# prtk1729/Paligemma-MultiModal-System

Measured on AMD Instinct MI355X. Metric: image→text tokens/sec + prefill ms, PaliGemma-3B-224 at 1/2/4/8 MI355X, higher is better.
Workload: dtype bf16; 1 GPU; PaliGemma-3B-pt-224 image->text, batch 1, prefill L=264, 128 greedy tokens (BASELINE.json configs[1]); global_batch=1, seq_len=392, parallelism=dp1, decode=hipgraph, prefill=eager

## Files before the change

### paligemma-multimodal-system_amd/csrc/common.h

```cpp
#pragma once
#include <hip/hip_runtime.h>
#include <stdint.h>

typedef uint16_t bf16_t;
typedef __attribute__((ext_vector_type(8))) __bf16 bf16x8;
typedef __attribute__((ext_vector_type(4))) float f32x4;
typedef __attribute__((ext_vector_type(2))) float f32x2;
typedef __attribute__((ext_vector_type(4))) uint32_t u32x4;
typedef __attribute__((ext_vector_type(2))) uint32_t u32x2;

#define LDS_AS __attribute__((address_space(3)))

__device__ __forceinline__ float bf2f(bf16_t v) { return __uint_as_float(((uint32_t)v) << 16); }

__device__ __forceinline__ bf16_t f2bf(float f) {
  __bf16 b = (__bf16)f;
  return __builtin_bit_cast(bf16_t, b);
}
typedef __bf16 pg_bf16x2_t __attribute__((ext_vector_type(2)));
typedef float pg_f32x2_t __attribute__((ext_vector_type(2)));
__device__ __forceinline__ uint32_t pack_bf2(float lo, float hi) {
  return __builtin_bit_cast(uint32_t, __builtin_convertvector(pg_f32x2_t{lo, hi}, pg_bf16x2_t));
}

__device__ __forceinline__ float bf_lo(uint32_t v) { return __uint_as_float(v << 16); }
__device__ __forceinline__ float bf_hi(uint32_t v) { return __uint_as_float(v & 0xffff0000u); }
__device__ __forceinline__ uint32_t pack_fp8x4(float a, float b, float c, float d) {
  int w = __builtin_amdgcn_cvt_pk_fp8_f32(fminf(fmaxf(a, -448.f), 448.f), fminf(fmaxf(b, -448.f), 448.f), 0, false);
  w = __builtin_amdgcn_cvt_pk_fp8_f32(fminf(fmaxf(c, -448.f), 448.f), fminf(fmaxf(d, -448.f), 448.f), w, true);
  return (uint32_t)w;
}

__device__ __forceinline__ float max_xor16(float v) {
  const auto r = __builtin_amdgcn_permlane16_swap(__float_as_uint(v), __float_as_uint(v), false, false);
  return fmaxf(__uint_as_float(r[0]), __uint_as_float(r[1]));
}
__device__ __forceinline__ float max_xor32(float v) {
  const auto r = __builtin_amdgcn_permlane32_swap(__float_as_uint(v), __float_as_uint(v), false, false);
  return fmaxf(__uint_as_float(r[0]), __uint_as_float(r[1]));
}
__device__ __forceinline__ float sum_xor16(float v) {
  const auto r = __builtin_amdgcn_permlane16_swap(__float_as_uint(v), __float_as_uint(v), false, false);
  return __uint_as_float(r[0]) + __uint_as_float(r[1]);
}
// ... 112 lines not shown
```

### paligemma-multimodal-system_amd/csrc/gemm.hip

```cpp
#include "gemm_common.h"

static int gemm_impl(const void* A, int lda, const void* W, int ldw, const float* bias, void* C, int ldc,
                     int M, int N, int K, int epi_flags, int ksplit, const float* aux, int aux_rows, void* aux_out,
                     int aux_ld, int aux_n, const PgFusedArgs* fa, hipStream_t stream) {
  const bool frag = (epi_flags & PG_W_FRAG) != 0;
  const bool fp8 = (epi_flags & PG_FP8) != 0;
  const bool m1 = (epi_flags & PG_TILE_M1) != 0;
  const bool n64 = (epi_flags & PG_TILE_N64) != 0;
  const int epi = epi_flags & 0xFF;
  const bool slot_rows = (epi_flags & PG_SLOT_ROWS) != 0;
  const bool frag13 = (epi_flags & PG_W_FRAG13) != 0;
  const bool frag12 = (epi_flags & PG_W_FRAG12) != 0;
  PG_REQUIRE((epi_flags & ~(0xFF | PG_W_FRAG | PG_FP8 | PG_TILE_M1 | PG_TILE_N64 | PG_SLOT_ROWS | PG_W_FRAG13 |
                            PG_W_FRAG12)) == 0 &&
             epi <= PG_EPI_F32_RES && (frag13 || !frag12));
  if (frag13) {
    const int pm = fa ? fa->pro_mode : 0;
    PG_REQUIRE(!frag && !fp8 && !m1 && !n64 && W != nullptr && ((uintptr_t)W & 15) == 0 && M >= 1 && M <= 4 &&
               N > 0 && N % 16 == 0 && K > 0 && K % 128 == 0 && ldw == K && ksplit >= 1 && ksplit <= 64 &&
               (K / 64) % (8 * ksplit) == 0);
    PG_REQUIRE((epi == PG_EPI_QKV_ROPE && pm == 1) || (epi == PG_EPI_BF16_GELU_MUL && pm == 1) ||
               (epi == PG_EPI_FX_ADD && (pm == 0 || pm == 2)) || (epi == PG_EPI_F32_FIN && pm == 0) ||
               (epi == PG_EPI_F32 && pm == 4));
  }
  if (m1) PG_REQUIRE(!fp8 && !n64 && M >= 256 && M <= 288 && (fa == nullptr || fa->pro_mode == 0));
  if (n64) PG_REQUIRE(M > 16);
  PG_REQUIRE(M > 0 && N > 0 && K > 0 && ksplit >= 1 && W != nullptr && C != nullptr);
  PG_REQUIRE(K % 32 == 0 && ldw >= K && (N % 4) == 0);
  if (frag && !fp8) PG_REQUIRE(N % 16 == 0 && K % 64 == 0 && ldw == K &&
                       (epi == PG_EPI_BF16 || epi == PG_EPI_BF16_GELU_MUL || epi == PG_EPI_F32 ||
                        epi == PG_EPI_QKV_ROPE || epi == PG_EPI_F32_FIN || epi == PG_EPI_F32_ADD ||
                        epi == PG_EPI_FX_ADD || epi == PG_EPI_F32_RES));
  PgFusedArgs f{};
// ... 98 lines not shown
```

### paligemma-multimodal-system_amd/csrc/gemm_gemv.hip

```cpp
#include "gemm_common.h"

#define XPAD 8

#ifndef PG_GEMV_PREW
#define PG_GEMV_PREW 1
#endif
#ifndef PG_GEMV_NT
#define PG_GEMV_NT 0
#endif
#ifndef PG_GEMV_CONTIG
#define PG_GEMV_CONTIG 0
#endif
#ifndef PG_GEMV_QKV_NT1
#define PG_GEMV_QKV_NT1 1
#endif
#ifndef PG_GEMV_D2
#define PG_GEMV_D2 4
#endif
#ifndef PG_GEMV_LM_NT
#define PG_GEMV_LM_NT 2
#endif
#ifndef PG_GEMV_LM_D
#define PG_GEMV_LM_D 6
#endif
// ... 300 lines not shown
  u32x4 cq;
  unsigned c5;
};
template <int MODE>
__device__ __forceinline__ void decode12(const W12& b, unsigned bias, u32x4 (&op)[2][2]) {
  unsigned q[4] = {b.cq[0], b.cq[1], b.cq[2], b.cq[3]};
  unsigned c5 = 0;
#pragma unroll
  for (int d = 0; d < 4; ++d) asm volatile("" : "+v"(q[d]));
  if constexpr (MODE > 0) {
    c5 = b.c5;
    asm volatile("" : "+v"(c5));
  }
  const unsigned badd = bias * 0x00800080u;
#pragma unroll
  for (int P = 0; P < 16; ++P) {
    const unsigned w = q[P >> 2];
    unsigned e = ((P & 3) == 0 ? w << 7 : (P & 3) == 1 ? w << 3 : (P & 3) == 2 ? w >> 1 : w >> 5) & 0x07800780u;
    if constexpr (MODE > 0)
      e |= (P < 11 ? c5 << (11 - P) : c5 >> (P - 11)) & 0x08000800u;
    if constexpr (MODE == 2) {
      const unsigned nz = ((e + 0x0f800f80u) >> 5) & 0x00800080u;
      e += __umul24(nz, bias);
    } else {
      e += badd;
    }
    const int h = P >> 3, s = (P >> 2) & 1, p = P & 3;
    const unsigned x = b.sm[h][p];
    const unsigned d = __builtin_amdgcn_perm(x, x, s == 0 ? 0x02020000u : 0x03030101u);
    op[h][s][p] = (d & 0x807f807fu) | e;
  }
}

template <int EPI, int NT, int U, int DEPTH, int PRO, int FRAG, int CPW = 0>
__device__ __forceinline__ void gemv_body(const bf16_t* __restrict__ A, int lda, const bf16_t* __restrict__ W,
                                          int ldw, int K, const EpiArgs& e, const GemvIdx gi) {
  constexpr int CH = U * 32;
  extern __shared__ __attribute__((aligned(16))) char dyn_smem[];
  const int lane = threadIdx.x & 63;
  const int wave = threadIdx.x >> 6;
  const int g = lane >> 4;
  const int r = lane & 15;
  const int tile0 = gi.bx * NT;
  const int M = e.M;
  const bool xvalid = r < M;

  const int z = gi.by;
  const int nch_all = K / CH;
  const int per_z = (nch_all + gi.ny - 1) / gi.ny;
  const int c0 = z * per_z;
  const int nch = min(nch_all - c0, per_z);
  const int mine = CPW > 0 ? CPW : (nch > wave ? (nch - wave + 3) / 4 : 0);
  constexpr int DB = DEPTH / 2;
  const int nb = CPW > 0 ? CPW / 2 : nch >> 3;

  const bf16_t* wrow[NT];
  const bf16_t* wfrag[NT];
#pragma unroll
  for (int t = 0; t < NT; ++t) {
    int n = (tile0 + t) * 16 + r;
    n = n < e.N ? n : e.N - 1;
    wrow[t] = W + (size_t)n * ldw;
    wfrag[t] = W + (size_t)min(tile0 + t, (e.N >> 4) - 1) * 16 * ldw;
  }
  f32x4 acc[NT];
#pragma unroll
  for (int t = 0; t < NT; ++t) acc[t] = f32x4{0.f, 0.f, 0.f, 0.f};

  bf16_t* xs = (bf16_t*)dyn_smem;
  const int Kr = per_z * CH;
  const bf16_t* xrow = (PRO == 0 || PRO == 4) ? A + (size_t)(xvalid ? r : M - 1) * lda : nullptr;
  constexpr bool SS16 = PRO == 4 && (NT >= 2 || EPI == PG_EPI_QKV_ROPE);
  constexpr int SSL = SS16 ? 16 : 4;
  float ssv[SSL];
#pragma unroll
  for (int k = 0; k < SSL; ++k) ssv[k] = 0.f;
  if constexpr (PRO == 4) {
    if (wave == 0) {
      if (SS16 && M > 2) {
        const int rr = min(r, M - 1);
#pragma unroll
        for (int k = 0; k < SSL; ++k) ssv[k] = e.f.ss_in[(size_t)rr * e.f.ss_ld + min(g + 4 * k, e.f.ss_n - 1)];
      } else {
        const int lpr = M == 1 ? 64 : 32;
        const int rr = min(lane / lpr, M - 1);
#pragma unroll
        for (int k = 0; k < 4; ++k) ssv[k] = e.f.ss_in[(size_t)rr * e.f.ss_ld + min(lane % lpr + k * lpr, e.f.ss_n - 1)];
      }
    }
  }
  const bf16_t* xlds = xs + (xvalid ? r : M - 1) * (Kr + XPAD);
  int rope_p = 0, rope_slot_raw = 0;
  if constexpr (EPI == PG_EPI_QKV_ROPE) {
    rope_p = e.f.pos[r < M ? r : M - 1];
    const int* slot_p = e.f.slot_dev ? e.f.slot_dev : &pg_zero_word;
    if (e.slot_rows) slot_p += (r < M ? r : M - 1) / e.f.rows_per_batch;
    rope_slot_raw = __hip_atomic_load(slot_p, __ATOMIC_RELAXED, __HIP_MEMORY_SCOPE_AGENT);
  }

  constexpr int S_STRIDE = PG_GEMV_CONTIG ? 32 : 8;
  const int LANE_OFF = PG_GEMV_CONTIG ? g * 8 : g * 8 * U;
  u32x4 wb[FRAG >= 2 ? 1 : DEPTH][NT][U];
  u32x4 xb[DEPTH][U];
  W13 wc[FRAG == 2 ? DB : 1][NT];
  constexpr int NTW = CPW > 0 ? CPW / 2 : DB;
  W12 wd[FRAG == 3 ? DB : 1][NT];
  unsigned tw[FRAG == 3 ? NT : 1][FRAG == 3 ? NTW : 1];
  unsigned twv[FRAG == 3 && CPW > 0 ? NT : 1][FRAG == 3 && CPW > 0 ? NTW : 1];
  const char* const w12 = (const char*)W;
  const size_t nblk12 = (size_t)(e.N >> 4) * (K >> 7);
  const unsigned* const tab12 = (const unsigned*)(w12 + nblk12 * PG_F12_BLOCK);
  const char* const heap12 = (const char*)tab12 + ((nblk12 * 4 + 255) & ~(size_t)255);
  auto blk12 = [&](int t, int i) {
    return (size_t)min(tile0 + t, (e.N >> 4) - 1) * (K >> 7) + ((c0 >> 3) + i) * 4 + wave;
  };
  if constexpr (FRAG == 3 && CPW > 0) {
#pragma unroll
    for (int i = 0; i < NTW; ++i)
#pragma unroll
      for (int t = 0; t < NT; ++t) twv[t][i] = tab12[blk12(t, i)];
    __builtin_amdgcn_sched_barrier(0);
  }
  auto loadm12 = [&](int i, W12 (&wv)[NT]) {
// ... 169 lines not shown
    float* scratch = (float*)(dyn_smem + (((size_t)M * (Kr + XPAD) * 2 + 15) & ~(size_t)15));
    if (PRO == 1 && PG_GEMV_PRO_EARLY && early)
      pro1_row_finish(e.f, K, p1, xs, scratch);
    else
      gemv_prologue<PRO>(e, M, K, c0 * CH, nch * CH, xs, scratch, A, lda, gi);
  }
#pragma unroll
  for (int d = 0; d < DEPTH; ++d) {
    if constexpr (FRAG == 2) {
      if (d < DB && (CPW > 0 ? d < CPW / 2 : d < nb)) {
        if (!prew) loadw13(d, wc[d]);
        loadx(2 * d, xb[2 * d]);
        loadx(2 * d + 1, xb[2 * d + 1]);
      }
      __builtin_amdgcn_sched_barrier(0);
    } else if constexpr (FRAG == 3) {
      if (d < DB && (CPW > 0 ? d < CPW / 2 : d < nb)) {
        if (!prew) {
          if constexpr (CPW > 0) loadm12(d, wd[d]);
          else loadw12(d, d, wd[d]);
        }
        loadx(2 * d, xb[2 * d]);
        loadx(2 * d + 1, xb[2 * d + 1]);
      }
      __builtin_amdgcn_sched_barrier(0);
    } else if (CPW > 0 ? d < CPW : d < mine) {
      if (!prew) loadw(d, wb[d]);
      loadx(d, xb[d]);
    }
  }
  if constexpr (FRAG == 3 && CPW > 0) {
    if (!prew) fifth12();
  }
  f32x4 fin_r[NT], fin_w[NT];
  i64x2 fin_fa[NT], fin_fb[NT];
  if constexpr (EPI == PG_EPI_F32_FIN) {
#pragma unroll
    for (int t = 0; t < NT; ++t) {
      const int n0 = min((tile0 + t) * 16, e.N - 16) + 4 * g;
      const size_t ro = (size_t)(r < M ? r : M - 1) * e.N + n0;
      fin_r[t] = *(const f32x4*)(e.f.fin_resid + ro);
      const long long* p = e.f.fx ? e.f.fx + ro : (const long long*)e.f.fin_resid;
      fin_fa[t] = *(const i64x2*)p;
      fin_fb[t] = *(const i64x2*)(p + 2);
      fin_w[t] = *(const f32x4*)((e.f.norm_w ? e.f.norm_w : e.f.fin_resid) + n0);
    }
  }
  f32x4 rope_cs[NT], rope_sn[NT];
  if constexpr (EPI == PG_EPI_QKV_ROPE) {
#pragma unroll
    for (int t = 0; t < NT; ++t) {
      bool roped;
      const int ii = rope_freq_index(e.f, min((tile0 + t) * 16, e.N - 16) + 4 * g, &roped);
      const long off = (long)rope_p * (e.f.head_dim >> 1) + ii;
      rope_cs[t] = *(const f32x4*)(e.f.cos_t + off);
      rope_sn[t] = *(const f32x4*)(e.f.sin_t + off);
    }
  }
  if constexpr (FRAG == 2 && CPW > 0) {
    __builtin_amdgcn_sched_barrier(0);
#pragma unroll
    for (int i = 0; i < CPW / 2; ++i) {
      const int d = i % DB;
      mfma13(wc[d], xb[2 * d], xb[2 * d + 1]);
      if (i + DB < CPW / 2) {
        loadw13(i + DB, wc[d]);
// ... 249 lines not shown
          if (e.bias && z == 0) v += load4_guard(e.bias, n0, e.N);
          if (e.f.resid_in && z == 0) v += load4_guard(e.f.resid_in + (size_t)m * e.N, n0, e.N);
          unsigned long long* dst = (unsigned long long*)e.C + (size_t)m * e.ldc + n0;
#pragma unroll
          for (int j = 0; j < 4; ++j) atomicAdd(dst + j, (unsigned long long)fx_from_f32_checked(v[j], e.f.status));
        }
      }
    }
    return;
  }
  if constexpr (EPI == PG_EPI_BF16_GELU_MUL) {
#pragma unroll
    for (int t = 0; t < NT; t += 2) epi_gelu_mul4(e, m, (tile0 + t) * 16, q, acc[t], acc[t + 1]);
  } else if constexpr (EPI == PG_EPI_QKV_ROPE) {
#pragma unroll
    for (int t = 0; t < NT; ++t) {
      f32x4 v = acc[t];
      const int n0 = (tile0 + t) * 16 + q;
      if (e.bias && n0 < e.N) v += load4_guard(e.bias, n0, e.N);
      f32x4 pr;
#pragma unroll
      for (int j = 0; j < 4; ++j) pr[j] = xchg_xor32(v[j]);
      epi_qkv_rope4_core(e, m, n0, v, pr, rope_cs[t], rope_sn[t], e.f.slot_base + rope_slot_raw);
    }
  } else {
#pragma unroll
    for (int t = 0; t < NT; ++t) epi_store4<EPI>(e, m, (tile0 + t) * 16 + q, acc[t], z);
  }
}

template <int EPI, int NT, int U, int DEPTH, int PRO, int FRAG, int CPW = 0>
__global__ __launch_bounds__(256)
__attribute__((amdgpu_waves_per_eu(FRAG >= 2 && CPW > 0 && EPI == PG_EPI_BF16_GELU_MUL ? 4 : 1, 8)))
void gemv_kernel(const bf16_t* __restrict__ A, int lda,
                                                   const bf16_t* __restrict__ W, int ldw, int K, EpiArgs e) {
  gemv_body<EPI, NT, U, DEPTH, PRO, FRAG, CPW>(A, lda, W, ldw, K, e,
                                               GemvIdx{(int)blockIdx.x, (int)blockIdx.y, (int)gridDim.x, (int)gridDim.y});
}

template <int EPI, int NT, int DEPTH, int PRO, bool FRAG>
static void launch_gemv_cpw(dim3 grid, size_t lds, hipStream_t st, const bf16_t* A, int lda, const bf16_t* W, int ldw,
                            int K, int ksplit, const EpiArgs& e) {
  const int nch = K / 64;
  const int cpw = (nch % ksplit == 0 && (nch / ksplit) % 4 == 0) ? nch / ksplit / 4 : 0;
  switch (PG_GEMV_CPW ? cpw : 0) {
    case 4: hipLaunchKernelGGL((gemv_kernel<EPI, NT, 2, DEPTH, PRO, FRAG, 4>), grid, dim3(256), lds, st, A, lda, W, ldw, K, e); break;
    case 8: hipLaunchKernelGGL((gemv_kernel<EPI, NT, 2, DEPTH, PRO, FRAG, 8>), grid, dim3(256), lds, st, A, lda, W, ldw, K, e); break;
    case 16: hipLaunchKernelGGL((gemv_kernel<EPI, NT, 2, DEPTH, PRO, FRAG, 16>), grid, dim3(256), lds, st, A, lda, W, ldw, K, e); break;
    default: hipLaunchKernelGGL((gemv_kernel<EPI, NT, 2, DEPTH, PRO, FRAG, 0>), grid, dim3(256), lds, st, A, lda, W, ldw, K, e); break;
  }
}

template <int EPI, int PRO, bool FRAG>
static void launch_gemv_pro(const bf16_t* A, int lda, const bf16_t* W, int ldw, int K, int ksplit, const EpiArgs& e,
                            hipStream_t st) {
  const int ntiles = (e.N + 15) / 16;
  const int CH = 64;
  const int per_z = (K / CH + ksplit - 1) / ksplit;
  size_t lds = 0;
  if ((PRO != 0 && PRO != 4) || PG_GEMV_XLDS) {
    lds = (size_t)e.M * (per_z * CH + XPAD) * 2;
    lds = (lds + 15) & ~(size_t)15;
    if (PRO == 1) lds += 64 * sizeof(float);
    if (PRO == 3) lds += 80 * sizeof(float);
  }
  if constexpr (PG_GEMV_QKV_NT1 && EPI == PG_EPI_QKV_ROPE) {
    if (e.M > 4) {
      launch_gemv_cpw<EPI, 1, PG_GEMV_D2, PRO, FRAG>(dim3(ntiles, ksplit), lds, st, A, lda, W, ldw, K, ksplit, e);
      return;
    }
  }
  if constexpr (PG_GEMV_LM_NT == 2 && EPI == PG_EPI_F32) {
    if (e.M <= 4 && ntiles >= 8192 && ksplit == 1) {
      launch_gemv_cpw<EPI, 2, PG_GEMV_LM_D, PRO, FRAG>(dim3((ntiles + 1) / 2, 1), lds, st, A, lda, W, ldw, K, 1, e);
      return;
    }
  }
  if constexpr (PG_GEMV_FIN_NT == 4 && EPI == PG_EPI_F32_FIN) {
    if (e.M > 4 && ntiles % 4 == 0) {
      launch_gemv_cpw<EPI, 4, PG_GEMV_D2, PRO, FRAG>(dim3(ntiles / 4, ksplit), lds, st, A, lda, W, ldw, K, ksplit, e);
      return;
    }
// ... 7 lines not shown

template <int EPI, bool FRAG>
static void launch_gemv(const bf16_t* A, int lda, const bf16_t* W, int ldw, int K, int ksplit, const EpiArgs& e,
                        hipStream_t st) {
  if constexpr (EPI == PG_EPI_F32_ADD || EPI == PG_EPI_FX_ADD) {
    if (e.f.pro_mode == 2)
      launch_gemv_pro<EPI, 2, FRAG>(A, lda, W, ldw, K, ksplit, e, st);
    else
      launch_gemv_pro<EPI, 0, FRAG>(A, lda, W, ldw, K, ksplit, e, st);
    return;
  }
  switch (e.f.pro_mode) {
    case 1: launch_gemv_pro<EPI, 1, FRAG>(A, lda, W, ldw, K, ksplit, e, st); break;
    case 2: launch_gemv_pro<EPI, 2, FRAG>(A, lda, W, ldw, K, ksplit, e, st); break;
    case 3: launch_gemv_pro<EPI, 3, FRAG>(A, lda, W, ldw, K, ksplit, e, st); break;
    case 4: launch_gemv_pro<EPI, 4, FRAG>(A, lda, W, ldw, K, ksplit, e, st); break;
    default: launch_gemv_pro<EPI, 0, FRAG>(A, lda, W, ldw, K, ksplit, e, st); break;
  }
}

template <int EPI, int NT, int DEPTH, int PRO, int F>
static void launch_gemv13(const bf16_t* A, int lda, const void* W, int K, int ksplit, const EpiArgs& e, hipStream_t st) {
  static_assert(DEPTH % 2 == 0, "whole blocks in flight");
  const int ntiles = e.N / 16;
  const int per_z = K / 64 / ksplit;
  size_t lds = 0;
  if (PRO != 0 && PRO != 4) {
    lds = (size_t)e.M * (per_z * 64 + XPAD) * 2;
    lds = (lds + 15) & ~(size_t)15;
    if (PRO == 1) lds += 64 * sizeof(float);
  }
  const dim3 grid((ntiles + NT - 1) / NT, ksplit);
  const bf16_t* w = (const bf16_t*)W;
  switch (PG_GEMV_CPW ? per_z / 4 : 0) {
    case 4: hipLaunchKernelGGL((gemv_kernel<EPI, NT, 2, DEPTH, PRO, F, 4>), grid, dim3(256), lds, st, A, lda, w, K, K, e); break;
    case 8: hipLaunchKernelGGL((gemv_kernel<EPI, NT, 2, DEPTH, PRO, F, 8>), grid, dim3(256), lds, st, A, lda, w, K, K, e); break;
    default: hipLaunchKernelGGL((gemv_kernel<EPI, NT, 2, DEPTH, PRO, F, 0>), grid, dim3(256), lds, st, A, lda, w, K, K, e); break;
  }
}

template <int F>
static int dispatch_gemv13(int epi, const bf16_t* A, int lda, const void* W, int K, int ksplit, const EpiArgs& e,
                           hipStream_t st) {
  const int pm = e.f.pro_mode;
  if (e.M > 4 || (K / 64) % (8 * ksplit)) return (int)hipErrorInvalidValue;
  if (epi == PG_EPI_QKV_ROPE && pm == 1) launch_gemv13<PG_EPI_QKV_ROPE, 1, PG_GEMV_D1, 1, F>(A, lda, W, K, ksplit, e, st);
  else if (epi == PG_EPI_FX_ADD && pm == 2) launch_gemv13<PG_EPI_FX_ADD, 1, PG_GEMV_D1, 2, F>(A, lda, W, K, ksplit, e, st);
  else if (epi == PG_EPI_FX_ADD && pm == 0) launch_gemv13<PG_EPI_FX_ADD, 1, PG_GEMV_D1, 0, F>(A, lda, W, K, ksplit, e, st);
  else if (epi == PG_EPI_F32_FIN && pm == 0) launch_gemv13<PG_EPI_F32_FIN, 1, PG_GEMV_D1, 0, F>(A, lda, W, K, ksplit, e, st);
  else if (epi == PG_EPI_BF16_GELU_MUL && pm == 1)
    launch_gemv13<PG_EPI_BF16_GELU_MUL, 2, PG_GEMV_D2, 1, F>(A, lda, W, K, ksplit, e, st);
  else if (epi == PG_EPI_F32 && pm == 4) launch_gemv13<PG_EPI_F32, 2, PG_GEMV_LM_D, 4, F>(A, lda, W, K, ksplit, e, st);
  else return (int)hipErrorInvalidValue;
  return 0;
}

int pg_dispatch_gemv13(int epi, int bits, const bf16_t* A, int lda, const void* W, int K, int ksplit, const EpiArgs& e,
                       hipStream_t st) {
  return bits == 12 ? dispatch_gemv13<3>(epi, A, lda, W, K, ksplit, e, st)
                    : dispatch_gemv13<2>(epi, A, lda, W, K, ksplit, e, st);
}

int pg_dispatch_gemv(int epi, bool frag, const bf16_t* A, int lda, const bf16_t* W, int ldw, int K, int ksplit,
                     const EpiArgs& e, hipStream_t st) {
#define PG_CASE(E)                                                                             \
  case E:                                                                                      \
    if (frag) launch_gemv<E, true>(A, lda, W, ldw, K, ksplit, e, st);                          \
    else launch_gemv<E, false>(A, lda, W, ldw, K, ksplit, e, st);                              \
    return 0;
#define PG_CASE_ROWMAJOR(E)                                                                    \
// ... 18 lines not shown
```

### paligemma-multimodal-system_amd/csrc/misc.hip

```cpp
#include <cstdlib>

#include "common.h"

__global__ void im2col_kernel(const float* __restrict__ px, int B, int C, int H, int W, int p, int nh, int nw,
                              bf16_t* __restrict__ out, int ldk) {
  const long total = (long)B * nh * nw * ldk;
  for (long i = blockIdx.x * (long)blockDim.x + threadIdx.x; i < total; i += (long)gridDim.x * blockDim.x) {
    const int col = (int)(i % ldk);
    const long row = i / ldk;
    const int pw = (int)(row % nw);
    const int ph = (int)((row / nw) % nh);
    const int b = (int)(row / ((long)nw * nh));
    float v = 0.f;
    if (col < C * p * p) {
      const int c = col / (p * p), kh = (col / p) % p, kw = col % p;
      v = px[(((long)b * C + c) * H + ph * p + kh) * W + pw * p + kw];
    }
    out[i] = f2bf(v);
  }
}

extern "C" int pg_patch_im2col(const float* px, int B, int C, int H, int W, int p, void* out, int ldk,
                               hipStream_t stream) {
  PG_REQUIRE(px && out && B > 0 && C > 0 && p > 0 && ldk >= C * p * p && H >= p && W >= p);
// ... 132 lines not shown
    vtc[((long)b * KV + cidx) * Smax + slot] = v[cidx];
}

extern "C" int pg_rope_kv_write(void* qkv, int ldq, const int* pos, int T, int L, int Hq, int Hkv, int D,
                                const float* cosT, const float* sinT, void* kc, void* vtc, int Smax, int slot_base,
                                const int* slot_dev, hipStream_t stream) {
  PG_REQUIRE(qkv && pos && cosT && sinT && kc && vtc && T > 0 && L > 0 && T % L == 0 && D % 2 == 0);
  hipLaunchKernelGGL(rope_kv_kernel, dim3(T), dim3(256), 0, stream, (bf16_t*)qkv, ldq, pos, L, Hq, Hkv, D, cosT, sinT,
                     (bf16_t*)kc, (bf16_t*)vtc, Smax, slot_base, slot_dev);
  PG_LAUNCH_CHECK();
  return 0;
}

#define AM_CHUNKS 64
__device__ __forceinline__ void am_better(float& bv, int& bi, float v, int i) {
  if (v > bv || (v == bv && i < bi)) { bv = v; bi = i; }
}
#define AM_NONE 0x7FFFFFFF
__device__ __forceinline__ int am_id(int bi) { return bi == AM_NONE ? 0 : bi; }
__device__ __forceinline__ void am_block(float& bv, int& bi, float* sv, int* si) {
  const int lane = threadIdx.x & 63, w = threadIdx.x >> 6;
#pragma unroll
  for (int o = 32; o > 0; o >>= 1) {
    float ov = __shfl_xor(bv, o, 64);
    int oi = __shfl_xor(bi, o, 64);
    am_better(bv, bi, ov, oi);
  }
  if (lane == 0) { sv[w] = bv; si[w] = bi; }
  __syncthreads();
  bv = sv[0]; bi = si[0];
  for (int i = 1; i < (int)(blockDim.x >> 6); ++i) am_better(bv, bi, sv[i], si[i]);
}

__global__ __launch_bounds__(256) void argmax_partial_kernel(const float* __restrict__ x, long ld, int V,
                                                             float* __restrict__ pv, int* __restrict__ pi) {
  __shared__ float sv[4];
  __shared__ int si[4];
  const int b = blockIdx.y, ch = blockIdx.x;
  const int per = ((V + AM_CHUNKS - 1) / AM_CHUNKS + 3) & ~3;
  const int s = ch * per, e = min(V, s + per);
  const float* row = x + (long)b * ld;
  float bv = -INFINITY;
  int bi = AM_NONE;
  for (int i = s + threadIdx.x * 4; i < e; i += 1024) {
    if (i + 3 < e) {
      const f32x4 v = *(const f32x4*)(row + i);
#pragma unroll
      for (int j = 0; j < 4; ++j) am_better(bv, bi, v[j], i + j);
    } else {
      for (int j = 0; j < 4 && i + j < e; ++j) am_better(bv, bi, row[i + j], i + j);
    }
  }
  am_block(bv, bi, sv, si);
  if (threadIdx.x == 0) { pv[b * AM_CHUNKS + ch] = bv; pi[b * AM_CHUNKS + ch] = bi; }
}

__global__ __launch_bounds__(1024) void argmax_final_kernel(const float* __restrict__ pv, const int* __restrict__ pi,
                                                            int B, int64_t* __restrict__ out_ids, int64_t* __restrict__ hist,
                                                            int hist_rows, int* __restrict__ step, int* __restrict__ pos,
                                                            int* __restrict__ kv_len) {
  const int lane = threadIdx.x & 63, wave = threadIdx.x >> 6, nw = blockDim.x >> 6;
  const int st = step ? *step : 0;
  __syncthreads();
  for (int b = wave; b < B; b += nw) {
    float bv = pv[b * AM_CHUNKS + lane];
    int bi = pi[b * AM_CHUNKS + lane];
#pragma unroll
    for (int o = 32; o > 0; o >>= 1) {
      float ov = __shfl_xor(bv, o, 64);
      int oi = __shfl_xor(bi, o, 64);
      am_better(bv, bi, ov, oi);
    }
    if (lane == 0) {
      bi = am_id(bi);
      out_ids[b] = bi;
      if (hist && st < hist_rows) hist[(long)st * B + b] = bi;
      if (pos) pos[b] += 1;
    }
  }
  if (threadIdx.x == 0) {
    if (kv_len) *kv_len += 1;
    if (step) *step = st + 1;
  }
}

#define AM_EMB_MAX_B 1024
struct AmEmbArgs {
  const bf16_t* embed;
  int V, n_feat, H;
  const float* feat;
  int64_t image_id, pad_id;
  float img_scale, normalizer;
  float* res;
};
__global__ __launch_bounds__(1024) void argmax_final_embed_kernel(const float* __restrict__ pv, const int* __restrict__ pi,
                                                                  int B, int64_t* __restrict__ out_ids,
                                                                  int64_t* __restrict__ hist, int hist_rows,
                                                                  int* __restrict__ step, int* __restrict__ pos,
                                                                  int* __restrict__ kv_len, AmEmbArgs ea) {
  __shared__ int win[AM_EMB_MAX_B];
  const int lane = threadIdx.x & 63, wave = threadIdx.x >> 6, nw = blockDim.x >> 6;
  const int st = step ? *step : 0;
  for (int b = wave; b < B; b += nw) {
    float bv = pv[b * AM_CHUNKS + lane];
    int bi = pi[b * AM_CHUNKS + lane];
#pragma unroll
    for (int o = 32; o > 0; o >>= 1) {
      float ov = __shfl_xor(bv, o, 64);
      int oi = __shfl_xor(bi, o, 64);
      am_better(bv, bi, ov, oi);
    }
    if (lane == 0) {
      bi = am_id(bi);
      win[b] = bi;
      out_ids[b] = bi;
      if (hist && st < hist_rows) hist[(long)st * B + b] = bi;
      if (pos) pos[b] += 1;
    }
  }
  __syncthreads();
  if (threadIdx.x == 0) {
    if (kv_len) *kv_len += 1;
    if (step) *step = st + 1;
  }
  for (int b = wave; b < B; b += nw) {
    const int64_t id = win[b];
    int rk = 0;
    if (id == ea.image_id)
      for (int i = 0; i < b; ++i) rk += win[i] == ea.image_id;
    embed_row(ea.res + (long)b * ea.H, id, rk, lane, 64, ea.embed, ea.V, ea.feat, ea.n_feat, ea.H, ea.image_id,
              ea.pad_id, ea.img_scale, ea.normalizer);
  }
// ... 11 lines not shown
    for (int o = 32; o > 0; o >>= 1) {
      float ov = __shfl_xor(bv, o, 64);
      int oi = __shfl_xor(bi, o, 64);
      am_better(bv, bi, ov, oi);
    }
    if (lane == 0) { pairs[2 * b] = bi == AM_NONE ? NAN : bv; pairs[2 * b + 1] = (float)(am_id(bi) + vocab_offset); }
  }
}

__global__ void argmax_merge_kernel(const float* __restrict__ pairs, int world, int B, int64_t* __restrict__ out_ids,
                                    int64_t* __restrict__ hist, int hist_rows, int* __restrict__ step, int* __restrict__ pos,
                                    int* __restrict__ kv_len) {
  if (threadIdx.x != 0) return;
  const int st = step ? *step : 0;
  for (int b = 0; b < B; ++b) {
    float bv = -INFINITY;
    int bi = AM_NONE;
    for (int r = 0; r < world; ++r) am_better(bv, bi, pairs[(r * B + b) * 2], (int)pairs[(r * B + b) * 2 + 1]);
    bi = am_id(bi);
    out_ids[b] = bi;
    if (hist && st < hist_rows) hist[(long)st * B + b] = bi;
    if (pos) pos[b] += 1;
  }
  if (kv_len) *kv_len += 1;
  if (step) *step = st + 1;
}

extern "C" int pg_argmax_pairs(const float* logits, long ld, int B, int V, int vocab_offset, void* workspace,
                               float* pairs, hipStream_t stream) {
  PG_REQUIRE(logits && workspace && pairs && B > 0 && V > 0 && ld % 4 == 0 && vocab_offset >= 0 &&
             vocab_offset + V < (1 << 24));
  float* pv = (float*)workspace;
  int* pi = (int*)(pv + B * AM_CHUNKS);
  hipLaunchKernelGGL(argmax_partial_kernel, dim3(AM_CHUNKS, B), dim3(256), 0, stream, logits, ld, V, pv, pi);
  hipLaunchKernelGGL(argmax_pairs_kernel, dim3(1), dim3(64 * am_waves(B)), 0, stream, pv, pi, B, vocab_offset, pairs);
  PG_LAUNCH_CHECK();
  return 0;
}

extern "C" int pg_argmax_merge(const float* pairs, int world, int B, int64_t* out_ids, int64_t* hist, int hist_rows,
                               int* step, int* pos, int* kv_len, hipStream_t stream) {
  PG_REQUIRE(pairs && out_ids && world > 0 && B > 0 && (hist == nullptr || hist_rows > 0));
  hipLaunchKernelGGL(argmax_merge_kernel, dim3(1), dim3(64), 0, stream, pairs, world, B, out_ids, hist, hist_rows,
                     step, pos, kv_len);
  PG_LAUNCH_CHECK();
  return 0;
}

extern "C" int pg_argmax(const float* logits, long ld, int B, int V, void* workspace, int64_t* out_ids,
                         int64_t* hist, int hist_rows, int* step, int* pos, int* kv_len, hipStream_t stream) {
  PG_REQUIRE(logits && workspace && out_ids && B > 0 && V > 0 && ld % 4 == 0 && (hist == nullptr || hist_rows > 0));
  float* pv = (float*)workspace;
  int* pi = (int*)(pv + B * AM_CHUNKS);
  hipLaunchKernelGGL(argmax_partial_kernel, dim3(AM_CHUNKS, B), dim3(256), 0, stream, logits, ld, V, pv, pi);
  hipLaunchKernelGGL(argmax_final_kernel, dim3(1), dim3(64 * am_waves(B)), 0, stream, pv, pi, B, out_ids, hist, hist_rows, step, pos,
                     kv_len);
  PG_LAUNCH_CHECK();
  return 0;
}

extern "C" int pg_argmax_embed(const float* logits, long ld, int B, int V, void* workspace, int64_t* out_ids,
                               int64_t* hist, int hist_rows, int* step, int* pos, int* kv_len, const void* embed,
                               int V_embed, const float* feat, int n_feat, int H, long image_id, long pad_id,
                               float img_scale, float normalizer, float* res, hipStream_t stream) {
  PG_REQUIRE(logits && workspace && out_ids && B > 0 && B <= AM_EMB_MAX_B && V > 0 && ld % 4 == 0 &&
             (hist == nullptr || hist_rows > 0));
  PG_REQUIRE(embed != nullptr && res != nullptr && V_embed > 0 && H > 0 && H % 4 == 0 && (n_feat == 0 || feat));
  float* pv = (float*)workspace;
  int* pi = (int*)(pv + B * AM_CHUNKS);
  const AmEmbArgs ea{(const bf16_t*)embed, V_embed, n_feat, H, feat, (int64_t)image_id, (int64_t)pad_id,
                     img_scale, normalizer, res};
  hipLaunchKernelGGL(argmax_partial_kernel, dim3(AM_CHUNKS, B), dim3(256), 0, stream, logits, ld, V, pv, pi);
  hipLaunchKernelGGL(argmax_final_embed_kernel, dim3(1), dim3(64 * am_waves(B)), 0, stream, pv, pi, B, out_ids, hist,
                     hist_rows, step, pos, kv_len, ea);
  PG_LAUNCH_CHECK();
  return 0;
}

__global__ __launch_bounds__(1024) void topp_kernel(const float* __restrict__ logits, long ld, int V, float inv_temp,
                                                    float top_p, const float* __restrict__ uniforms,
                                                    int64_t* __restrict__ out_ids, int64_t* __restrict__ hist, int hist_rows,
                                                    int* __restrict__ step, int* __restrict__ pos, int B,
                                                    int* __restrict__ kv_len, float* __restrict__ probs_out) {
  __shared__ float red[16];
  __shared__ float hist_mass[256];
  __shared__ float scan[1024];
  __shared__ int sel;
  __shared__ float sel_above;
  const int b = blockIdx.x;
  const float* x = logits + (long)b * ld;
  const int tid = threadIdx.x;
  float mx = -INFINITY;
  for (int i = tid; i < V; i += 1024) mx = fmaxf(mx, x[i] * inv_temp);
  mx = wave_max(mx);
  if ((tid & 63) == 0) red[tid >> 6] = mx;
  __syncthreads();
  mx = red[0];
  for (int i = 1; i < 16; ++i) mx = fmaxf(mx, red[i]);
  __syncthreads();
  float z = 0.f;
  for (int i = tid; i < V; i += 1024) z += __expf(x[i] * inv_temp - mx);
  z = block_sum(z, red);
  const float target = top_p * z;
  uint32_t prefix = 0;
  float above = 0.f;
  for (int digit = 3; digit >= 0; --digit) {
    const int shift = digit * 8;
// ... 391 lines not shown
```

### paligemma-multimodal-system_amd/pghip/build.py

```python
from __future__ import annotations

import concurrent.futures as cf
import glob
import hashlib
import os
import re
import subprocess
import sys

HERE = os.path.dirname(os.path.abspath(__file__))
PKG = os.path.dirname(HERE)
CSRC = os.path.join(PKG, "csrc")
INCLUDE = os.path.join(os.path.dirname(PKG), "include")
LIB = os.path.join(HERE, "libpghip.so")
OBJ_ROOT = os.path.join(PKG, "build", "obj")
ARCH = os.environ.get("PGHIP_ARCH", "gfx950")
HIPCC = os.environ.get("HIPCC", "/opt/rocm/bin/hipcc")
FLAGS = ["-O3", f"--offload-arch={ARCH}", "-fPIC", "-std=c++17", "-I", CSRC, "-I", INCLUDE,
         "-Wno-pass-failed"]
_MARK = b"PGHIP_SOURCE_HASH="


def sources():
    return sorted(glob.glob(os.path.join(CSRC, "*.hip")))


def _inputs():
    return sources() + sorted(glob.glob(os.path.join(CSRC, "*.h"))) + [os.path.join(INCLUDE, "pghip.h")]


def _config() -> str:
    flags = [f for f in FLAGS if f not in (CSRC, INCLUDE)]
    return " ".join([os.path.basename(HIPCC), *flags])


def _config_tag(defines=()) -> str:
    return hashlib.sha256(" ".join([_config(), *defines]).encode()).hexdigest()[:12]


def source_hash(defines=()) -> str:
    h = hashlib.sha256()
    for p in _inputs():
        h.update(os.path.relpath(p, os.path.dirname(PKG)).encode() + b"\0")
        with open(p, "rb") as f:
            h.update(f.read())
        h.update(b"\0")
    h.update(" ".join([_config(), *defines]).encode())
    return h.hexdigest()


def library_hash(path: str = LIB):
    if not os.path.exists(path):
        return None
    with open(path, "rb") as f:
        data = f.read()
    m = re.search(re.escape(_MARK) + rb"([0-9a-f]{64}|unknown)", data)
    return m.group(1).decode() if m else None


def _stale(defines=()) -> bool:
    return library_hash() != source_hash(defines)


def _obj_key(src: str, defines=()) -> str:
    h = hashlib.sha256()
    for p in [src] + sorted(glob.glob(os.path.join(CSRC, "*.h"))):
        with open(p, "rb") as f:
            h.update(os.path.basename(p).encode() + b"\0" + f.read() + b"\0")
    h.update(" ".join([_config(), *defines]).encode())
    return h.hexdigest()[:20]


def _compile(src: str, obj: str, defines=()) -> str:
    cmd = [HIPCC, *FLAGS, *[f"-D{d}" for d in defines], "-c", src, "-o", obj + ".tmp"]
    r = subprocess.run(cmd, capture_output=True, text=True)
    if r.returncode != 0:
        raise RuntimeError(f"hipcc failed on {src}:\n{r.stderr}")
    os.replace(obj + ".tmp", obj)
    return obj


def build(force: bool = False, verbose: bool = True, out: str = LIB, defines=()) -> str:
    if out == LIB and not defines and not force and not _stale():
        return LIB
    obj_dir = os.path.join(OBJ_ROOT, _config_tag(defines))
    os.makedirs(obj_dir, exist_ok=True)
    srcs = sources()
    jobs = min(len(srcs), int(os.environ.get("MAX_JOBS", os.cpu_count() or 4)), 16)
    shash = source_hash(defines)
    hash_def = f'PG_SOURCE_HASH="{shash}"'

    def obj_for(src):
        base = os.path.basename(src)
        if base == "misc.hip":
            return _compile(src, os.path.join(obj_dir, base + ".o"), (*defines, hash_def))
        obj = os.path.join(obj_dir, f"{base}.{_obj_key(src, defines)}.o")
        if force or not os.path.exists(obj):
            for old in glob.glob(os.path.join(obj_dir, base + ".*.o")):
                os.remove(old)
            return _compile(src, obj, defines)
        return obj
    with cf.ThreadPoolExecutor(max_workers=max(1, jobs)) as ex:
        objs = list(ex.map(obj_for, srcs))
    tmp = out + ".tmp"
    cmd = [HIPCC, f"--offload-arch={ARCH}", "-shared", "-fPIC", *objs, "-o", tmp]
    r = subprocess.run(cmd, capture_output=True, text=True)
    if r.returncode != 0:
# ... 11 lines not shown
```

Before: 1056 tokens/s.

## Enable kernarg preloading and reorder hot kernel arguments into preload slots

Compiles gemm_gemv.hip and misc.hip with the AMDGPU kernarg preload option (16 SGPRs). Kernel signatures are reordered so the most-used scalars and pointers come first and get preloaded, and large structs are moved to the end or passed as a struct. A new gemv_hot_kernel variant passes the hot pointers and sizes as leading scalars, and a launch helper chooses it for some forms. The aim is to cut kernel-start latency from kernarg loads in the many small decode GEMV and argmax kernels. The cost is extra kernel variants, more SGPR pressure, and an ABI change that is guarded by static_asserts.

```diff
diff --git a/paligemma-multimodal-system_amd/csrc/common.h b/paligemma-multimodal-system_amd/csrc/common.h
--- a/paligemma-multimodal-system_amd/csrc/common.h
+++ b/paligemma-multimodal-system_amd/csrc/common.h
@@ -10,6 +10,10 @@
 typedef __attribute__((ext_vector_type(2))) uint32_t u32x2;
 
 #define LDS_AS __attribute__((address_space(3)))
+
+#ifndef PG_KARG_HOT
+#define PG_KARG_HOT 1
+#endif
 
 __device__ __forceinline__ float bf2f(bf16_t v) { return __uint_as_float(((uint32_t)v) << 16); }
 
diff --git a/paligemma-multimodal-system_amd/csrc/gemm.hip b/paligemma-multimodal-system_amd/csrc/gemm.hip
--- a/paligemma-multimodal-system_amd/csrc/gemm.hip
+++ b/paligemma-multimodal-system_amd/csrc/gemm.hip
@@ -1,4 +1,6 @@
 #include "gemm_common.h"
+
+static_assert(sizeof(PgFusedArgs) == 336 && sizeof(EpiArgs) == 408, "PgFusedArgs / EpiArgs layout (ABI 13)");
 
 static int gemm_impl(const void* A, int lda, const void* W, int ldw, const float* bias, void* C, int ldc,
                      int M, int N, int K, int epi_flags, int ksplit, const float* aux, int aux_rows, void* aux_out,
diff --git a/paligemma-multimodal-system_amd/csrc/gemm_gemv.hip b/paligemma-multimodal-system_amd/csrc/gemm_gemv.hip
--- a/paligemma-multimodal-system_amd/csrc/gemm_gemv.hip
+++ b/paligemma-multimodal-system_amd/csrc/gemm_gemv.hip
@@ -356,7 +356,7 @@
   }
 }
 
-template <int EPI, int NT, int U, int DEPTH, int PRO, int FRAG, int CPW = 0>
+template <int EPI, int NT, int U, int DEPTH, int PRO, int FRAG, int CPW = 0, bool HOT = false>
 __device__ __forceinline__ void gemv_body(const bf16_t* __restrict__ A, int lda, const bf16_t* __restrict__ W,
                                           int ldw, int K, const EpiArgs& e, const GemvIdx gi) {
   constexpr int CH = U * 32;
@@ -399,7 +399,7 @@
   float ssv[SSL];
 #pragma unroll
   for (int k = 0; k < SSL; ++k) ssv[k] = 0.f;
-  if constexpr (PRO == 4) {
+  auto load_ss = [&]() {
     if (wave == 0) {
       if (SS16 && M > 2) {
         const int rr = min(r, M - 1);
@@ -412,7 +412,8 @@
         for (int k = 0; k < 4; ++k) ssv[k] = e.f.ss_in[(size_t)rr * e.f.ss_ld + min(lane % lpr + k * lpr, e.f.ss_n - 1)];
       }
     }
-  }
+  };
+  if constexpr (PRO == 4 && !HOT) load_ss();
   const bf16_t* xlds = xs + (xvalid ? r : M - 1) * (Kr + XPAD);
   int rope_p = 0, rope_slot_raw = 0;
   if constexpr (EPI == PG_EPI_QKV_ROPE) {
@@ -648,6 +649,7 @@
   if constexpr (FRAG == 3 && CPW > 0) {
     if (!prew) fifth12();
   }
+  if constexpr (PRO == 4 && HOT) load_ss();
   f32x4 fin_r[NT], fin_w[NT];
   i64x2 fin_fa[NT], fin_fb[NT];
   if constexpr (EPI == PG_EPI_F32_FIN) {
@@ -963,10 +965,48 @@
 template <int EPI, int NT, int U, int DEPTH, int PRO, int FRAG, int CPW = 0>
 __global__ __launch_bounds__(256)
 __attribute__((amdgpu_waves_per_eu(FRAG >= 2 && CPW > 0 && EPI == PG_EPI_BF16_GELU_MUL ? 4 : 1, 8)))
-void gemv_kernel(const bf16_t* __restrict__ A, int lda,
-                                                   const bf16_t* __restrict__ W, int ldw, int K, EpiArgs e) {
+void gemv_kernel(EpiArgs e, const bf16_t* __restrict__ A, int lda, const bf16_t* __restrict__ W, int ldw, int K) {
   gemv_body<EPI, NT, U, DEPTH, PRO, FRAG, CPW>(A, lda, W, ldw, K, e,
                                                GemvIdx{(int)blockIdx.x, (int)blockIdx.y, (int)gridDim.x, (int)gridDim.y});
+}
+
+template <int EPI, int NT, int U, int DEPTH, int PRO, int FRAG, int CPW = 0>
+__global__ __launch_bounds__(256)
+__attribute__((amdgpu_waves_per_eu(FRAG >= 2 && CPW > 0 && EPI == PG_EPI_BF16_GELU_MUL ? 4 : 1, 8)))
+void gemv_hot_kernel(const bf16_t* __restrict__ W, const void* h0, const void* h1, const void* h2,
+                     unsigned long long x3, int N, int K, int mf, int ldw, const bf16_t* __restrict__ A, int lda,
+                     EpiArgs e) {
+  static_assert(PRO == 0 || PRO == 1 || PRO == 4, "forms with a header");
+  EpiArgs eh = e;
+  eh.N = N;
+  eh.M = mf & 0xffff;
+  if constexpr (PRO == 1) {
+    eh.f.fx = (long long*)h0;
+    eh.f.resid_in = (const float*)h1;
+    eh.f.norm_w = (const float*)h2;
+  } else {
+    A = (const bf16_t*)h0;
+    lda = (int)x3;
+    eh.f.ss_in = (const float*)h2;
+  }
+  gemv_body<EPI, NT, U, DEPTH, PRO, FRAG, CPW, true>(
+      A, lda, W, ldw, K, eh, GemvIdx{(int)blockIdx.x, (int)blockIdx.y, 0, (int)((unsigned)mf >> 16)});
+}
+
+template <bool HOT, int EPI, int NT, int DEPTH, int PRO, int FRAG, int CPW>
+static void launch_gemv_one(dim3 grid, size_t lds, hipStream_t st, const bf16_t* A, int lda, const bf16_t* W, int ldw,
+                            int K, const EpiArgs& e) {
+  if constexpr (HOT && PG_KARG_HOT) {
+    const PgFusedArgs& f = e.f;
+    const void *h0 = nullptr, *h1 = nullptr, *h2 = nullptr;
+    unsigned long long x3 = 0;
+    if (PRO == 1) h0 = f.fx, h1 = f.resid_in, h2 = f.norm_w;
+    else h0 = A, h2 = f.ss_in, x3 = (unsigned)lda;
+    hipLaunchKernelGGL((gemv_hot_kernel<EPI, NT, 2, DEPTH, PRO, FRAG, CPW>), grid, dim3(256), lds, st, W, h0, h1, h2, x3,
+                       e.N, K, (int)(e.M | grid.y << 16), ldw, A, lda, e);
+  } else {
+    hipLaunchKernelGGL((gemv_kernel<EPI, NT, 2, DEPTH, PRO, FRAG, CPW>), grid, dim3(256), lds, st, e, A, lda, W, ldw, K);
+  }
 }
 
 template <int EPI, int NT, int DEPTH, int PRO, bool FRAG>
@@ -975,10 +1015,10 @@
   const int nch = K / 64;
   const int cpw = (nch % ksplit == 0 && (nch / ksplit) % 4 == 0) ? nch / ksplit / 4 : 0;
   switch (PG_GEMV_CPW ? cpw : 0) {
-    case 4: hipLaunchKernelGGL((gemv_kernel<EPI, NT, 2, DEPTH, PRO, FRAG, 4>), grid, dim3(256), lds, st, A, lda, W, ldw, K, e); break;
-    case 8: hipLaunchKernelGGL((gemv_kernel<EPI, NT, 2, DEPTH, PRO, FRAG, 8>), grid, dim3(256), lds, st, A, lda, W, ldw, K, e); break;
-    case 16: hipLaunchKernelGGL((gemv_kernel<EPI, NT, 2, DEPTH, PRO, FRAG, 16>), grid, dim3(256), lds, st, A, lda, W, ldw, K, e); break;
-    default: hipLaunchKernelGGL((gemv_kernel<EPI, NT, 2, DEPTH, PRO, FRAG, 0>), grid, dim3(256), lds, st, A, lda, W, ldw, K, e); break;
+    case 4: launch_gemv_one<false, EPI, NT, DEPTH, PRO, FRAG, 4>(grid, lds, st, A, lda, W, ldw, K, e); break;
+    case 8: launch_gemv_one<false, EPI, NT, DEPTH, PRO, FRAG, 8>(grid, lds, st, A, lda, W, ldw, K, e); break;
+    case 16: launch_gemv_one<false, EPI, NT, DEPTH, PRO, FRAG, 16>(grid, lds, st, A, lda, W, ldw, K, e); break;
+    default: launch_gemv_one<false, EPI, NT, DEPTH, PRO, FRAG, 0>(grid, lds, st, A, lda, W, ldw, K, e); break;
   }
 }
 
@@ -1052,10 +1092,11 @@
   }
   const dim3 grid((ntiles + NT - 1) / NT, ksplit);
   const bf16_t* w = (const bf16_t*)W;
+  constexpr bool HOT = PRO == 0 || PRO == 4 || EPI == PG_EPI_BF16_GELU_MUL;
   switch (PG_GEMV_CPW ? per_z / 4 : 0) {
-    case 4: hipLaunchKernelGGL((gemv_kernel<EPI, NT, 2, DEPTH, PRO, F, 4>), grid, dim3(256), lds, st, A, lda, w, K, K, e); break;
-    case 8: hipLaunchKernelGGL((gemv_kernel<EPI, NT, 2, DEPTH, PRO, F, 8>), grid, dim3(256), lds, st, A, lda, w, K, K, e); break;
-    default: hipLaunchKernelGGL((gemv_kernel<EPI, NT, 2, DEPTH, PRO, F, 0>), grid, dim3(256), lds, st, A, lda, w, K, K, e); break;
+    case 4: launch_gemv_one<HOT, EPI, NT, DEPTH, PRO, F, 4>(grid, lds, st, A, lda, w, K, K, e); break;
+    case 8: launch_gemv_one<HOT, EPI, NT, DEPTH, PRO, F, 8>(grid, lds, st, A, lda, w, K, K, e); break;
+    default: launch_gemv_one<HOT, EPI, NT, DEPTH, PRO, F, 0>(grid, lds, st, A, lda, w, K, K, e); break;
   }
 }
 
diff --git a/paligemma-multimodal-system_amd/csrc/misc.hip b/paligemma-multimodal-system_amd/csrc/misc.hip
--- a/paligemma-multimodal-system_amd/csrc/misc.hip
+++ b/paligemma-multimodal-system_amd/csrc/misc.hip
@@ -188,8 +188,19 @@
   for (int i = 1; i < (int)(blockDim.x >> 6); ++i) am_better(bv, bi, sv[i], si[i]);
 }
 
-__global__ __launch_bounds__(256) void argmax_partial_kernel(const float* __restrict__ x, long ld, int V,
-                                                             float* __restrict__ pv, int* __restrict__ pi) {
+struct AmPartArgs {
+  const float* x;
+  long ld;
+  int V;
+  float* pv;
+  int* pi;
+};
+__global__ __launch_bounds__(256) void argmax_partial_kernel(AmPartArgs a) {
+  const float* __restrict__ x = a.x;
+  const long ld = a.ld;
+  const int V = a.V;
+  float* __restrict__ pv = a.pv;
+  int* __restrict__ pi = a.pi;
   __shared__ float sv[4];
   __shared__ int si[4];
   const int b = blockIdx.y, ch = blockIdx.x;
@@ -249,11 +260,19 @@
   float img_scale, normalizer;
   float* res;
 };
+#if PG_KARG_HOT
+__global__ __launch_bounds__(1024) void argmax_final_embed_kernel(const float* __restrict__ pv, const int* __restrict__ pi,
+                                                                  int* __restrict__ step, int64_t* __restrict__ out_ids,
+                                                                  int64_t* __restrict__ hist, int* __restrict__ pos,
+                                                                  int B, int hist_rows,
+                                                                  int* __restrict__ kv_len, AmEmbArgs ea) {
+#else
 __global__ __launch_bounds__(1024) void argmax_final_embed_kernel(const float* __restrict__ pv, const int* __restrict__ pi,
                                                                   int B, int64_t* __restrict__ out_ids,
                                                                   int64_t* __restrict__ hist, int hist_rows,
                                                                   int* __restrict__ step, int* __restrict__ pos,
                                                                   int* __restrict__ kv_len, AmEmbArgs ea) {
+#endif
   __shared__ int win[AM_EMB_MAX_B];
   const int lane = threadIdx.x & 63, wave = threadIdx.x >> 6, nw = blockDim.x >> 6;
   const int st = step ? *step : 0;
@@ -331,7 +350,7 @@
              vocab_offset + V < (1 << 24));
   float* pv = (float*)workspace;
   int* pi = (int*)(pv + B * AM_CHUNKS);
-  hipLaunchKernelGGL(argmax_partial_kernel, dim3(AM_CHUNKS, B), dim3(256), 0, stream, logits, ld, V, pv, pi);
+  hipLaunchKernelGGL(argmax_partial_kernel, dim3(AM_CHUNKS, B), dim3(256), 0, stream, AmPartArgs{logits, ld, V, pv, pi});
   hipLaunchKernelGGL(argmax_pairs_kernel, dim3(1), dim3(64 * am_waves(B)), 0, stream, pv, pi, B, vocab_offset, pairs);
   PG_LAUNCH_CHECK();
   return 0;
@@ -351,7 +370,7 @@
   PG_REQUIRE(logits && workspace && out_ids && B > 0 && V > 0 && ld % 4 == 0 && (hist == nullptr || hist_rows > 0));
   float* pv = (float*)workspace;
   int* pi = (int*)(pv + B * AM_CHUNKS);
-  hipLaunchKernelGGL(argmax_partial_kernel, dim3(AM_CHUNKS, B), dim3(256), 0, stream, logits, ld, V, pv, pi);
+  hipLaunchKernelGGL(argmax_partial_kernel, dim3(AM_CHUNKS, B), dim3(256), 0, stream, AmPartArgs{logits, ld, V, pv, pi});
   hipLaunchKernelGGL(argmax_final_kernel, dim3(1), dim3(64 * am_waves(B)), 0, stream, pv, pi, B, out_ids, hist, hist_rows, step, pos,
                      kv_len);
   PG_LAUNCH_CHECK();
@@ -369,9 +388,14 @@
   int* pi = (int*)(pv + B * AM_CHUNKS);
   const AmEmbArgs ea{(const bf16_t*)embed, V_embed, n_feat, H, feat, (int64_t)image_id, (int64_t)pad_id,
                      img_scale, normalizer, res};
-  hipLaunchKernelGGL(argmax_partial_kernel, dim3(AM_CHUNKS, B), dim3(256), 0, stream, logits, ld, V, pv, pi);
+  hipLaunchKernelGGL(argmax_partial_kernel, dim3(AM_CHUNKS, B), dim3(256), 0, stream, AmPartArgs{logits, ld, V, pv, pi});
+#if PG_KARG_HOT
+  hipLaunchKernelGGL(argmax_final_embed_kernel, dim3(1), dim3(64 * am_waves(B)), 0, stream, pv, pi, step, out_ids, hist,
+                     pos, B, hist_rows, kv_len, ea);
+#else
   hipLaunchKernelGGL(argmax_final_embed_kernel, dim3(1), dim3(64 * am_waves(B)), 0, stream, pv, pi, B, out_ids, hist,
                      hist_rows, step, pos, kv_len, ea);
+#endif
   PG_LAUNCH_CHECK();
   return 0;
 }
diff --git a/paligemma-multimodal-system_amd/pghip/build.py b/paligemma-multimodal-system_amd/pghip/build.py
--- a/paligemma-multimodal-system_amd/pghip/build.py
+++ b/paligemma-multimodal-system_amd/pghip/build.py
@@ -18,6 +18,8 @@
 HIPCC = os.environ.get("HIPCC", "/opt/rocm/bin/hipcc")
 FLAGS = ["-O3", f"--offload-arch={ARCH}", "-fPIC", "-std=c++17", "-I", CSRC, "-I", INCLUDE,
          "-Wno-pass-failed"]
+PRELOAD_FLAGS = ["-mllvm", "-amdgpu-kernarg-preload-count=16"]
+PRELOAD_SOURCES = ("gemm_gemv.hip", "misc.hip")
 _MARK = b"PGHIP_SOURCE_HASH="
 
 
@@ -31,7 +33,7 @@
 
 def _config() -> str:
     flags = [f for f in FLAGS if f not in (CSRC, INCLUDE)]
-    return " ".join([os.path.basename(HIPCC), *flags])
+    return " ".join([os.path.basename(HIPCC), *flags, *PRELOAD_FLAGS, "@", *PRELOAD_SOURCES])
 
 
 def _config_tag(defines=()) -> str:
@@ -72,7 +74,8 @@
 
 
 def _compile(src: str, obj: str, defines=()) -> str:
-    cmd = [HIPCC, *FLAGS, *[f"-D{d}" for d in defines], "-c", src, "-o", obj + ".tmp"]
+    extra = PRELOAD_FLAGS if os.path.basename(src) in PRELOAD_SOURCES else []
+    cmd = [HIPCC, *FLAGS, *extra, *[f"-D{d}" for d in defines], "-c", src, "-o", obj + ".tmp"]
     r = subprocess.run(cmd, capture_output=True, text=True)
     if r.returncode != 0:
         raise RuntimeError(f"hipcc failed on {src}:\n{r.stderr}")
```

After: 1068 tokens/s (median of 6 runs). +1.1%, better.
